# cg-tuwien/ppsurf

Measured on AMD Instinct MI355X. Metric: occupancy query-points/sec @ res=257, 50NN, higher is better.
Workload: dtype f16x3

## Files before the change

### include/ppsurf_amd_ext.h

```cpp
#ifndef PPSURF_AMD_EXT_H
#define PPSURF_AMD_EXT_H
#include <stddef.h>
#include <stdint.h>

#ifdef __cplusplus
extern "C" {
#endif

int ppsx_blend_rgba_u8(const int64_t* idx, const float* d2, int64_t m, int k, const uint8_t* rgba, int64_t n, double eps, uint8_t* out,
                       void* stream);

int ppsx_trim_cell_slots(const float* pts, int64_t n, const float* lo, const float* hi, float h, float inv_h, uint64_t* table, int64_t capacity,
                         int64_t* slot, void* stream);
int ppsx_trim_face_support(const float* verts, int64_t nv, const int64_t* faces, int64_t nf, const float* pts, int64_t n, const float* lo,
                           const float* hi, float h, float inv_h, const uint64_t* table, int64_t capacity, const int64_t* order,
                           const int64_t* offsets, double r, uint8_t* support, void* stream);

int ppsx_smooth_half_edges(const int64_t* faces, int64_t nf, int64_t nv, int64_t* keys, void* stream);
int ppsx_smooth_pass(const double* x, int64_t nv, const int64_t* offsets, const int32_t* nbr, const int32_t* mult, int64_t ne, double s,
                     double* out, void* stream);

int ppsx_normals_corner_keys(const int64_t* faces, int64_t nf, int64_t nv, int64_t* keys, void* stream);
int ppsx_normals_vertex(const float* verts, int64_t nv, const int64_t* faces, int64_t nf, const int64_t* offsets, const int32_t* inc, int64_t ni,
                        int weight, float* out, void* stream);
// ... 4 lines not shown
                       int64_t* keys, void* stream);
int ppsx_fill_loops(const int64_t* cand, int64_t nc, const int32_t* succ, int64_t nv, int max_edges, int32_t* len, void* stream);
int ppsx_fill_emit(const float* verts, int64_t nv, const int32_t* succ, const int64_t* leader, const int32_t* len, const int64_t* vslot,
                   const int64_t* foff, int64_t nl, float* new_verts, int64_t nnew, int64_t* new_faces, int64_t nfnew, void* stream);

int ppsx_denoise_face_normals(const float* verts, int64_t nv, const int64_t* faces, int64_t nf, double* normals, void* stream);
int ppsx_denoise_filter_pass(const int64_t* faces, int64_t nf, int64_t nv, const int64_t* offsets, const int32_t* inc, int64_t ni,
                             const double* normals, double threshold, double* out, void* stream);
int ppsx_denoise_vertex_pass(const double* x, int64_t nv, const int64_t* faces, int64_t nf, const double* normals, const int64_t* offsets,
                             const int32_t* inc, int64_t ni, double* out, void* stream);

int ppsx_pieces_edge_keys(const int64_t* faces, int64_t nf, int64_t nv, int64_t* keys, void* stream);
int ppsx_pieces_hook(const int32_t* fa, const int32_t* fb, int64_t np, int32_t* label, int64_t nf, int32_t* changed, void* stream);
int ppsx_pieces_compress(int32_t* label, int64_t nf, void* stream);
int ppsx_pieces_stats(const float* verts, int64_t nv, const int64_t* faces, int64_t nf, const int32_t* label, const int32_t* cid, int64_t nc,
                      int64_t* count, float* lo, float* hi, void* stream);
int ppsx_pieces_select(const int64_t* count, const float* lo, const float* hi, const int64_t* rank, int64_t nc, int has_min_faces,
                       int64_t min_faces, int has_min_diag_frac, double min_diag_frac, int has_keep_largest, int64_t keep_largest,
                       double box_diag2, uint8_t* keep, void* stream);

int ppsx_decimate_regular(const int64_t* offsets, const int32_t* mult, int64_t ne, const int64_t* inc_offsets, int64_t ni, int64_t nv,
                          uint8_t* regular, void* stream);
int ppsx_decimate_edges(const double* pos, int64_t nv, const int64_t* faces, int64_t nf, const int64_t* offsets, const int32_t* nbr,
                        const int32_t* src, int64_t ne, const int64_t* inc_offsets, const int32_t* inc, int64_t ni, const uint8_t* regular,
                        uint64_t* prio, double* x, uint8_t* fell, void* stream);
int ppsx_decimate_vertex_min(const int64_t* offsets, const int32_t* nbr, int64_t ne, int64_t nv, const uint64_t* prio, uint64_t* m1, void* stream);
int ppsx_decimate_ring_min(const int64_t* offsets, const int32_t* nbr, int64_t ne, int64_t nv, const uint64_t* m1, uint64_t* best, void* stream);
int ppsx_decimate_winners(const int32_t* src, const int32_t* nbr, int64_t ne, int64_t nv, const uint64_t* prio, const uint64_t* best, uint8_t* flag,
                          void* stream);
int ppsx_decimate_move(const int64_t* win, int64_t nw, const int32_t* src, const int32_t* nbr, int64_t ne, const double* x, double* pos, int64_t nv,
                       int32_t* rename, void* stream);
int ppsx_decimate_rename(const int64_t* faces, int64_t nf, int64_t nv, const int32_t* rename, int64_t* out, uint8_t* keep, void* stream);

#ifdef __cplusplus
}
#endif
#endif
```

### ppsurf_amd/csrc/pps_decode.hip

```cpp
#include <cstdlib>
#include "pps_common.h"
#include "../../include/ppsurf_amd.h"

using namespace pps;

#define NT 256
#define NW (NT / 64)
#define WG_PER_CU (512 / NT)
#ifndef PPS_PRIO
#define PPS_PRIO 1
#endif
#ifndef PPS_PRIO_PN
#define PPS_PRIO_PN 1
#endif
#define CH4 2048

template <int CHUNK_F4_NEXT, int NTH = NT, class F>
__device__ __forceinline__ void stream_step(const f32x4* __restrict__ gnext, f32x4*& cur, f32x4*& nxt, F&& compute) {
    chunk_copy_async<CHUNK_F4_NEXT / NTH, NTH>(gnext, nxt);
    compute((const f32x4*)cur);
    stream_wait();
    __syncthreads();
    f32x4* t = cur; cur = nxt; nxt = t;
}
// ... 1133 lines not shown
    f32x4 *cur, *nxt;
    stream_begin<CH4>(wg, cur, nxt);

    const int ntiles = (int)((Q + NW * 16 - 1) / (NW * 16));
    int first, count, stride;
    xcd_tile_range(ntiles, first, count, stride);
    for (int it = 0; it < count; ++it) {
        const TileRow q = tile_row(first + it * stride, wave, n, Q);
        f32x4 p[16], x[8], h[16];
        {
            const f32x4* sp = (const f32x4*)(pooled + q.c * 256) + g;
            const f32x4* sx = (const f32x4*)(xbar + q.c * 128) + g;
#pragma unroll
            for (int bb = 0; bb < 16; ++bb) p[bb] = sp[4 * bb];
#pragma unroll
            for (int bb = 0; bb < 8; ++bb) x[bb] = sx[4 * bb];
        }
#pragma unroll
        for (int c = 0; c < 8; ++c)
            stream_step<CH4>(wg + (c + 1) * CH4, cur, nxt,
                           [&](const f32x4* w) { dense_blocks<16, 2, 0>(p, &h[2 * c], w, bias4 + 8 * c, lane); });
#pragma unroll
        for (int c = 0; c < 4; ++c)
            stream_step<CH4>(wg + (c + 9) * CH4, cur, nxt,
                           [&](const f32x4* w) { dense_blocks<8, 4, 1, 1>(x, &h[4 * c], w, bias4, lane); });
#pragma unroll
        for (int c = 0; c < 8; ++c)
            stream_step<CH4>(wg + (c + 13) * CH4, cur, nxt,
                           [&](const f32x4* w) { dense_blocks<16, 2, 1>(h, &p[2 * c], w, bias4 + 64 + 8 * c, lane); });
        f32x4 o[2];
        stream_step<CH4>(wg, cur, nxt, [&](const f32x4* w) { dense_blocks<16, 2, 0>(p, o, w, bias4 + 128, lane); });
        store_logits(o[0], q, g, logits, occ);
    }
}

__global__ __launch_bounds__(NT, 2) void decode_tail_h_kernel(const float* __restrict__ pooled, const float* __restrict__ xbar, int64_t Q,
                                                              const f32x4* __restrict__ w16, const float* __restrict__ bias,
                                                              float* __restrict__ logits, float* __restrict__ occ, int* __restrict__ range) {
    float amax = 0.f;
    float* bias_l = (float*)((f32x4*)pps_smem + 2 * CH4);
    const f32x4* bias4 = (const f32x4*)bias_l;
    const f32x4* wg = w16;
    const int lane = lane_id(), wave = threadIdx.x >> 6, n = lane & 15, g = lane >> 4;

    lds_fill(bias_l, bias, TL_NBIAS);
    f32x4 *cur, *nxt;
    stream_begin<CH4>(wg, cur, nxt);

    const int ntiles = (int)((Q + NW * 16 - 1) / (NW * 16));
    int first, count, stride;
    xcd_tile_range(ntiles, first, count, stride);
    for (int it = 0; it < count; ++it) {
        const TileRow q = tile_row(first + it * stride, wave, n, Q);
        HiLo p[8], x[4];
        {
            const f32x4* sp = (const f32x4*)(pooled + q.c * 256) + g;
            const f32x4* sx = (const f32x4*)(xbar + q.c * 128) + g;
#pragma unroll
            for (int kb = 0; kb < 8; ++kb) p[kb] = split_f16_r(amax, sp[4 * (2 * kb)], sp[4 * (2 * kb + 1)]);
#pragma unroll
            for (int kb = 0; kb < 4; ++kb) x[kb] = split_f16_r(amax, sx[4 * (2 * kb)], sx[4 * (2 * kb + 1)]);
        }
        HiLo y[8];
#pragma unroll
        for (int c = 0; c < 8; ++c) {
            f32x4 h[2];
// ... 212 lines not shown
                        float* logits, float* occ, void* stream) {
    return decode_tail_f32_impl(pooled, xbar, q, wpack, bias, logits, occ, nullptr, stream);
}

int pps_decode_tail_f16x3(const float* pooled, const float* xbar, int64_t q, const void* w16, const float* bias, float* logits, float* occ,
                          int32_t* range_flag, void* stream) {
    if (q < 0) return PPS_ERR_ARG;
    if (q == 0) return PPS_OK;
    if (!pooled || !xbar || !w16 || !bias || !logits) return PPS_ERR_ARG;
    return launch<decode_tail_h_kernel>(grid_for((q + NW * 16 - 1) / (NW * 16)), NT, TL_LDS_BYTES, stream, pooled, xbar, q, (const f32x4*)w16, bias,
                                        logits, occ, (int*)range_flag);
}

#define PPS_DECODE_WS_HEAD 64
size_t pps_decode_ws_bytes(int64_t q) { return q < 0 ? 0 : (size_t)q * (256 + 256 + 4096 + 256) * sizeof(float) + PPS_DECODE_WS_HEAD; }

static int decode_fwd(const float* table, const float* pts, const float* query, const int64_t* idx, int64_t q, int k,
                      const float* patches, int p, const float* const* weights, float* logits, float* occ, void* ws, void* const* events,
                      void* stream, const void* const* w16 = nullptr) {
    const void* interp_w16 = w16 ? w16[0] : nullptr;
    const bool pn16 = w16 && w16[1] && w16[2] && w16[3];
    if (q < 0) return PPS_ERR_ARG;
    if (q == 0) return PPS_OK;
    if (!weights || !ws || !logits) return PPS_ERR_ARG;
    for (int i = 0; i < 10; ++i)
        if (!weights[i]) return PPS_ERR_ARG;
    int* guard = (int*)ws;
    float* pooled = (float*)ws + PPS_DECODE_WS_HEAD / sizeof(float);
    float* g = pooled + q * 256;
    float* trans2 = g + q * 256;
    float* xbar = trans2 + q * 4096;
    hipStream_t st = (hipStream_t)stream;
    const bool split = interp_w16 || pn16 || (w16 && w16[4]);
    if (split && hipMemsetAsync(guard, 0, sizeof(int), st) != hipSuccess) return PPS_ERR_LAUNCH;
#define PPS_MARK(i) do { if (events && events[i] && hipEventRecord((hipEvent_t)events[i], st) != hipSuccess) return PPS_ERR_LAUNCH; } while (0)
    PPS_MARK(0);
    int rc = interp_w16 ? pps_interp_pool_f16x3(table, pts, query, idx, q, k, weights[0], interp_w16, weights[1], pooled, guard, stream)
                        : pps_interp_pool_f32(table, pts, query, idx, q, k, weights[0], weights[1], pooled, stream);
    PPS_MARK(1);
    if (pn16) {
        if (rc == PPS_OK) rc = pps_pointnet_f16x3(patches, q, p, weights + 2, w16 + 1, g, trans2, xbar, guard, events ? events + 2 : nullptr, stream);
    } else {
        if (rc == PPS_OK) rc = pps_pointnet_stn_rows_f32(patches, q, p, weights[2], weights[3], g, stream);
        PPS_MARK(2);
        if (rc == PPS_OK) rc = pps_pointnet_stn_fc_f32(g, q, weights[4], weights[5], trans2, stream);
        PPS_MARK(3);
        if (rc == PPS_OK) rc = pps_pointnet_feat_rows_f32(patches, trans2, q, p, weights[6], weights[7], xbar, stream);
        PPS_MARK(4);
    }
    if (rc == PPS_OK)
        rc = (w16 && w16[4]) ? pps_decode_tail_f16x3(pooled, xbar, q, w16[4], weights[9], logits, occ, guard, stream)
                             : pps_decode_tail_f32(pooled, xbar, q, weights[8], weights[9], logits, occ, stream);
    PPS_MARK(5);
#undef PPS_MARK
    if (split && rc == PPS_OK) {
        rc = interp_pool_f32_impl(table, pts, query, idx, q, k, weights[0], weights[1], pooled, guard, stream);
        if (rc == PPS_OK) rc = launch_stn_rows<false>(patches, q, p, weights[2], weights[2] + PA_W_XYZ, weights[3], g, guard, stream);
        if (rc == PPS_OK) rc = stn_fc_f32_impl(g, q, weights[4], weights[5], trans2, guard, stream);
        if (rc == PPS_OK) rc = launch_feat_rows<false>(patches, trans2, q, p, weights[6], weights[6] + PC_W_XYZ, weights[7], xbar, guard, stream);
        if (rc == PPS_OK) rc = decode_tail_f32_impl(pooled, xbar, q, weights[8], weights[9], logits, occ, guard, stream);
    }
    return rc;
}

int pps_decode_fwd_f32(const float* table, const float* pts, const float* query, const int64_t* idx, int64_t q, int k,
                       const float* patches, int p, const float* const* weights, float* logits, float* occ, void* ws, void* stream) {
    return decode_fwd(table, pts, query, idx, q, k, patches, p, weights, logits, occ, ws, nullptr, stream);
// ... 17 lines not shown
```

### ppsurf_amd/csrc/pps_knn.hip

```cpp
#include "pps_common.h"
#include "../../include/ppsurf_amd.h"

#define KNN_QW 8
#define KNN_WAVES 4
#define KNN_CAP 128
#ifndef KNN_BISECT
#define KNN_BISECT 12
#endif
#ifndef KNN_SEED
#define KNN_SEED 4
#endif

typedef unsigned long long u64;

__device__ __forceinline__ u64 shfl_xor_u64(u64 v, int m) {
    const int lo = __shfl_xor((int)(unsigned)v, m), hi = __shfl_xor((int)(unsigned)(v >> 32), m);
    return ((u64)(unsigned)hi << 32) | (unsigned)lo;
}
__device__ __forceinline__ u64 shfl_u64(u64 v, int src) {
    const int lo = __shfl((int)(unsigned)v, src), hi = __shfl((int)(unsigned)(v >> 32), src);
    return ((u64)(unsigned)hi << 32) | (unsigned)lo;
}

__device__ __forceinline__ float wave_min_f32(float v, int lane) {
    v = fminf(v, pps::dpp_mov<0xB1>(v));
    v = fminf(v, pps::dpp_mov<0x4E>(v));
    v = fminf(v, pps::dpp_mov<0x141>(v));
    v = fminf(v, pps::dpp_mov<0x140>(v));
    v = fminf(v, __uint_as_float(pps::lane_xor_u32(__float_as_uint(v), 16, lane)));
    v = fminf(v, __uint_as_float(pps::lane_xor_u32(__float_as_uint(v), 32, lane)));
    return v;
}

__device__ __forceinline__ u64 wave_sort64(u64 key, int lane) {
#pragma unroll
    for (int size = 2; size <= 64; size <<= 1) {
#pragma unroll
        for (int st = size >> 1; st > 0; st >>= 1) {
            const u64 other = pps::lane_xor_u64(key, st, lane);
            const bool up = ((lane & size) == 0);
            const bool lower = ((lane & st) == 0);
            const bool take_min = (up == lower);
            const u64 mn = key < other ? key : other, mx = key < other ? other : key;
            key = take_min ? mn : mx;
        }
    }
    return key;
}
__device__ __forceinline__ u64 wave_bitonic_merge64(u64 key, int lane) {
#pragma unroll
    for (int st = 32; st > 0; st >>= 1) {
        const u64 other = pps::lane_xor_u64(key, st, lane);
        const bool lower = ((lane & st) == 0);
        const u64 mn = key < other ? key : other, mx = key < other ? other : key;
        key = lower ? mn : mx;
    }
    return key;
}

__device__ __forceinline__ u64 knn_flush(u64 list, const u64* cand, int cnt, int lane) {
    while (cnt > 0) {
        const int c = cnt < 64 ? cnt : 64;
        u64 ck = (lane < c) ? cand[cnt - c + lane] : ~0ull;
        ck = wave_sort64(ck, lane);
        const u64 rev = shfl_u64(ck, 63 - lane);
        list = wave_bitonic_merge64(list < rev ? list : rev, lane);
        cnt -= c;
    }
    return list;
}

__global__ __launch_bounds__(KNN_WAVES * 64) void knn_kernel(const float* __restrict__ pts, int n, const float* __restrict__ query,
                                                             int64_t m, int k, int64_t* __restrict__ out_idx,
                                                             float* __restrict__ out_d2) {
    __shared__ u64 cand_all[KNN_WAVES][KNN_QW][KNN_CAP];
    const int lane = threadIdx.x & 63, wave = threadIdx.x >> 6;
    const int64_t ntask = (m + KNN_QW - 1) / KNN_QW;
    for (int64_t task = (int64_t)blockIdx.x * KNN_WAVES + wave; task < ntask; task += (int64_t)gridDim.x * KNN_WAVES) {
        const int64_t q0 = task * KNN_QW;
        float qx[KNN_QW], qy[KNN_QW], qz[KNN_QW], tau[KNN_QW];
        u64 list[KNN_QW];
        int cnt[KNN_QW];
#pragma unroll
        for (int j = 0; j < KNN_QW; ++j) {
            const int64_t qq = (q0 + j < m) ? q0 + j : m - 1;
            qx[j] = __builtin_nontemporal_load(query + qq * 3);
            qy[j] = query[qq * 3 + 1];
            qz[j] = query[qq * 3 + 2];
// ... 26 lines not shown
                }
            }
        }
#pragma unroll
        for (int j = 0; j < KNN_QW; ++j) {
            list[j] = knn_flush(list[j], cand_all[wave][j], cnt[j], lane);
            if (q0 + j < m && lane < k) {
                out_idx[(q0 + j) * k + lane] = (int64_t)(unsigned)(list[j] & 0xffffffffull);
                if (out_d2) out_d2[(q0 + j) * k + lane] = __uint_as_float((unsigned)(list[j] >> 32));
            }
        }
    }
}

__device__ __forceinline__ void wave_merge2(u64& a, u64& b, int lane) {
    const u64 rev = shfl_u64(b, 63 - lane);
    const u64 lo = a < rev ? a : rev, hi = a < rev ? rev : a;
    a = wave_bitonic_merge64(lo, lane);
    b = wave_bitonic_merge64(hi, lane);
}

template <int R>
__device__ __forceinline__ void knn_flush_r(u64 (&list)[R], const u64* cand, int cnt, int lane) {
    while (cnt > 0) {
        const int c = cnt < 64 ? cnt : 64;
        u64 carry = (lane < c) ? cand[cnt - c + lane] : ~0ull;
        carry = wave_sort64(carry, lane);
#pragma unroll
        for (int r = 0; r < R; ++r) wave_merge2(list[r], carry, lane);
        cnt -= c;
    }
}

template <int R>
__global__ __launch_bounds__(KNN_WAVES * 64) void knn_blocked_kernel(const float* __restrict__ pts, const int* __restrict__ orig,
                                                                     const float* __restrict__ bbox, int nb,
                                                                     const float* __restrict__ win_bbox, int n_win,
                                                                     const float* __restrict__ sbox ,
                                                                     const float* __restrict__ query, int64_t m, int k,
                                                                     int64_t* __restrict__ out_idx, float* __restrict__ out_d2) {
    __shared__ u64 cand_all[KNN_WAVES][KNN_QW][KNN_CAP];
    const int ngrp = (nb + 63) >> 6;
    const int lane = threadIdx.x & 63, wave = threadIdx.x >> 6;
    const int kr = (k - 1) >> 6, kl = (k - 1) & 63;
    const int64_t ntask = (m + KNN_QW - 1) / KNN_QW;
    for (int64_t task = (int64_t)blockIdx.x * KNN_WAVES + wave; task < ntask; task += (int64_t)gridDim.x * KNN_WAVES) {
        const int64_t q0 = task * KNN_QW;
        float qx[KNN_QW], qy[KNN_QW], qz[KNN_QW], tau[KNN_QW];
        u64 list[KNN_QW][R];
        int cnt[KNN_QW], wbest[KNN_QW];
#pragma unroll
        for (int j = 0; j < KNN_QW; ++j) {
            const int64_t qq = (q0 + j < m) ? q0 + j : m - 1;
            qx[j] = __shfl(query[qq * 3], 0); qy[j] = __shfl(query[qq * 3 + 1], 0); qz[j] = __shfl(query[qq * 3 + 2], 0);
            tau[j] = INFINITY;
            wbest[j] = 0;
#pragma unroll
            for (int r = 0; r < R; ++r) list[j][r] = ~0ull;
            cnt[j] = 0;
        }
        if (sbox != nullptr && n_win > 0) {
#pragma unroll
            for (int j = 0; j < KNN_QW; ++j) {
                float best = INFINITY;
                int bw = 0;
                for (int g0 = 0; g0 * 64 < n_win; g0 += 64) {
                    const int g = g0 + lane;
                    const bool gv = g * 64 < n_win;
                    const float* gb = sbox + (int64_t)(gv ? g : 0) * 6;
                    const float gx = fmaxf(fmaxf(__fsub_rn(gb[0], qx[j]), __fsub_rn(qx[j], gb[3])), 0.f);
                    const float gy = fmaxf(fmaxf(__fsub_rn(gb[1], qy[j]), __fsub_rn(qy[j], gb[4])), 0.f);
                    const float gz = fmaxf(fmaxf(__fsub_rn(gb[2], qz[j]), __fsub_rn(qz[j], gb[5])), 0.f);
                    const float gnear = gv ? __fadd_rn(__fadd_rn(__fmul_rn(gx, gx), __fmul_rn(gy, gy)), __fmul_rn(gz, gz)) : INFINITY;
// ... 12 lines not shown
                        const float tf = wave_min_f32(far2, lane);
                        if (tf < best) {
                            best = tf;
                            bw = (g0 + src) * 64 + __builtin_ctzll(__ballot(far2 == tf));
                        }
                        pend &= ~(1ull << src);
                        pend &= __ballot(gnear < best);
                    }
                }
                tau[j] = best;
                wbest[j] = bw;
            }
        } else {
            for (int b0 = 0; b0 < n_win; b0 += 64) {
                const int b = b0 + lane;
                const bool bv = b < n_win;
                const float* bb = win_bbox + (int64_t)(bv ? b : 0) * 6;
                const float lx = bb[0], ly = bb[1], lz = bb[2], hx = bb[3], hy = bb[4], hz = bb[5];
#pragma unroll
                for (int j = 0; j < KNN_QW; ++j) {
                    const float fx = fmaxf(fabsf(__fsub_rn(qx[j], lx)), fabsf(__fsub_rn(qx[j], hx)));
                    const float fy = fmaxf(fabsf(__fsub_rn(qy[j], ly)), fabsf(__fsub_rn(qy[j], hy)));
                    const float fz = fmaxf(fabsf(__fsub_rn(qz[j], lz)), fabsf(__fsub_rn(qz[j], hz)));
                    const float far2 = bv ? __fadd_rn(__fadd_rn(__fmul_rn(fx, fx), __fmul_rn(fy, fy)), __fmul_rn(fz, fz)) : INFINITY;
                    if (far2 < tau[j]) { tau[j] = far2; wbest[j] = b; }
                }
            }
        }
        const int nfull = n_win > 0 ? n_win + R - 1 : 0;
        constexpr int SEEDS = KNN_SEED > R ? KNN_SEED : R;
        const int nseed = nfull < SEEDS ? nfull : SEEDS;
#pragma unroll
        for (int j = 0; j < KNN_QW; ++j) {
            const float t = wave_min_f32(tau[j], lane);
            const u64 who = __ballot(tau[j] == t);
            tau[j] = t;
            if (nseed > 0) {
                const int w = __shfl(wbest[j], who != 0ull ? __builtin_ctzll(who) : 0);
                int s0 = w - (nseed - R) / 2;
                s0 = s0 < 0 ? 0 : s0;
                s0 = s0 + nseed > nfull ? nfull - nseed : s0;
                unsigned u[SEEDS];
#pragma unroll
                for (int rr = 0; rr < SEEDS; ++rr) {
                    const int p = (s0 + (rr < nseed ? rr : 0)) * 64 + lane;
                    const float dx = __fsub_rn(qx[j], pts[3 * p]), dy = __fsub_rn(qy[j], pts[3 * p + 1]), dz = __fsub_rn(qz[j], pts[3 * p + 2]);
                    const float d2 = __fadd_rn(__fadd_rn(__fmul_rn(dx, dx), __fmul_rn(dy, dy)), __fmul_rn(dz, dz));
                    u[rr] = rr < nseed ? __float_as_uint(d2) : 0xffffffffu;
                }
                unsigned lo = 0u, hi = __float_as_uint(tau[j]);
                {
                    int c = 0;
#pragma unroll
                    for (int rr = 0; rr < SEEDS; ++rr) c += __popcll(__ballot(u[rr] <= hi));
                    if (c < k) lo = hi;
                }
#pragma unroll
                for (int it = 0; it < KNN_BISECT; ++it) {
                    const unsigned mid = lo + ((hi - lo) >> 1);
                    int c = 0;
#pragma unroll
                    for (int rr = 0; rr < SEEDS; ++rr) c += __popcll(__ballot(u[rr] <= mid));
                    if (c >= k) hi = mid; else lo = mid + (lo < hi ? 1u : 0u);
                }
                tau[j] = __uint_as_float(hi);
            }
        }
// ... 56 lines not shown
                    const float d2 = __fadd_rn(__fadd_rn(__fmul_rn(dx, dx), __fmul_rn(dy, dy)), __fmul_rn(dz, dz));
                    const bool pass = pv && (d2 <= tau[j]);
                    const u64 mask = __ballot(pass);
                    if (mask != 0ull) {
                        u64* cand = cand_all[wave][j];
                        const int pos = cnt[j] + (int)__builtin_amdgcn_mbcnt_hi((unsigned)(mask >> 32), __builtin_amdgcn_mbcnt_lo((unsigned)mask, 0));
                        if (pass) cand[pos] = ((u64)__float_as_uint(d2) << 32) | (unsigned)oi;
                        cnt[j] += __popcll(mask);
                        if (cnt[j] > KNN_CAP - 64) {
                            knn_flush_r<R>(list[j], cand + (cnt[j] - 64), 64, lane);
                            cnt[j] -= 64;
                            u64 kth = list[j][R - 1];
#pragma unroll
                            for (int r = 0; r + 1 < R; ++r) kth = (r == kr) ? list[j][r] : kth;
                            tau[j] = fminf(tau[j], __uint_as_float((unsigned)(shfl_u64(kth, kl) >> 32)));
                        }
                    }
                }
            }
          }
        }
#pragma unroll
        for (int j = 0; j < KNN_QW; ++j) {
            knn_flush_r<R>(list[j], cand_all[wave][j], cnt[j], lane);
            if (q0 + j < m) {
#pragma unroll
                for (int r = 0; r < R; ++r) {
                    const int e = r * 64 + lane;
                    if (e < k) {
                        out_idx[(q0 + j) * k + e] = (int64_t)(unsigned)(list[j][r] & 0xffffffffull);
                        if (out_d2) out_d2[(q0 + j) * k + e] = __uint_as_float((unsigned)(list[j][r] >> 32));
                    }
                }
            }
        }
    }
}

#define KBB_MAX 8
struct KbbKind {
    const float* pts; const int* orig; const float* bbox; const float* win; const float* query; const int* q_orig; int64_t* out;
    int64_t pts_stride, orig_stride, bbox_stride, win_stride, query_stride, qorig_stride, out_stride;
    int nb, n_win, m, k, groups, group_end;
};
struct KbbArgs { KbbKind kind[KBB_MAX]; int nkinds, nclouds; };

__global__ __launch_bounds__(KNN_WAVES * 64) void knn_blocked_batch_kernel(const KbbArgs a) {
    __shared__ u64 cand_all[KNN_WAVES][KNN_QW][KNN_CAP];
    const int lane = threadIdx.x & 63, wave = threadIdx.x >> 6;
    const int total = a.kind[a.nkinds - 1].group_end;
    for (int grp = blockIdx.x * KNN_WAVES + wave; grp < total; grp += gridDim.x * KNN_WAVES) {
        int t = 0;
        while (grp >= a.kind[t].group_end) ++t;
        const KbbKind& kd = a.kind[t];
        const int local = grp - (t == 0 ? 0 : a.kind[t - 1].group_end);
        const int cloud = local / kd.groups, q0 = (local % kd.groups) * KNN_QW;
        const float* __restrict__ pts = kd.pts + cloud * kd.pts_stride;
        const int* __restrict__ orig = kd.orig + cloud * kd.orig_stride;
        const float* __restrict__ bbox = kd.bbox + cloud * kd.bbox_stride;
        const float* __restrict__ win_bbox = kd.win + cloud * kd.win_stride;
        const float* __restrict__ query = kd.query + cloud * kd.query_stride;
        const int nb = kd.nb, n_win = kd.n_win, m = kd.m, k = kd.k;
        float qx[KNN_QW], qy[KNN_QW], qz[KNN_QW], tau[KNN_QW];
        u64 list[KNN_QW];
        int cnt[KNN_QW];
#pragma unroll
        for (int j = 0; j < KNN_QW; ++j) {
            const int qq = (q0 + j < m) ? q0 + j : m - 1;
            qx[j] = __shfl(query[qq * 3], 0); qy[j] = __shfl(query[qq * 3 + 1], 0); qz[j] = __shfl(query[qq * 3 + 2], 0);
// ... 117 lines not shown
}

int pps_knn_blocked_f32(const float* pts_blocked, const int32_t* orig_idx, const float* bbox, int64_t nb, int64_t n,
                        const float* win_bbox, int64_t n_win, const float* query, int64_t m, int k, int64_t* out_idx, float* out_d2,
                        void* stream) {
    return pps_knn_blocked_groups_f32(pts_blocked, orig_idx, bbox, nb, n, win_bbox, n_win, nullptr, query, m, k, out_idx, out_d2, stream);
}

int pps_knn_blocked_groups_f32(const float* pts_blocked, const int32_t* orig_idx, const float* bbox, int64_t nb, int64_t n,
                               const float* win_bbox, int64_t n_win, const float* group_bbox, const float* query, int64_t m, int k,
                               int64_t* out_idx, float* out_d2, void* stream) {
    if (n < 1 || nb < 1 || nb * 64 < n || (nb - 1) * 64 >= n || m < 0 || k < 1 || k > 256 || k > n || nb > 0x1ffffff || n_win < 0)
        return PPS_ERR_ARG;
    if (m == 0) return PPS_OK;
    if (!pts_blocked || !orig_idx || !bbox || !query || !out_idx || (n_win > 0 && !win_bbox)) return PPS_ERR_ARG;
    const int64_t ntask = (m + KNN_QW - 1) / KNN_QW;
    int64_t blocks = (ntask + KNN_WAVES - 1) / KNN_WAVES;
    int cus = pps_device_cu_count();
    if (cus <= 0) cus = 256;
    if (blocks > (int64_t)cus * 8) blocks = (int64_t)cus * 8;
    const dim3 grid((unsigned)blocks), block(KNN_WAVES * 64);
    hipStream_t st = (hipStream_t)stream;
    const int r = (k + 63) / 64;
#define PPS_KNN_LAUNCH(R) hipLaunchKernelGGL(knn_blocked_kernel<R>, grid, block, 0, st, pts_blocked, orig_idx, bbox, (int)nb, win_bbox, \
                                             (int)n_win, group_bbox, query, m, k, out_idx, out_d2)
    if (r == 1) PPS_KNN_LAUNCH(1);
    else if (r == 2) PPS_KNN_LAUNCH(2);
    else if (r == 3) PPS_KNN_LAUNCH(3);
    else PPS_KNN_LAUNCH(4);
#undef PPS_KNN_LAUNCH
    return hipGetLastError() == hipSuccess ? PPS_OK : PPS_ERR_LAUNCH;
}

int pps_knn_blocked_batch_f32(int nkinds, int64_t nclouds, const float* const* pts_blocked, const int32_t* const* orig_idx,
                              const float* const* bbox, const int64_t* nb, const float* const* win_bbox, const int64_t* n_win,
                              const float* const* query, const int32_t* const* q_orig, const int64_t* query_stride, const int64_t* m,
                              const int* k, int64_t* const* out_idx, void* stream) {
    if (nkinds < 1 || nkinds > KBB_MAX || nclouds < 1 || !pts_blocked || !orig_idx || !bbox || !nb || !win_bbox || !n_win || !query || !q_orig ||
        !query_stride || !m || !k || !out_idx)
        return PPS_ERR_ARG;
    KbbArgs a;
    int64_t total = 0;
    for (int t = 0; t < nkinds; ++t) {
        if (!pts_blocked[t] || !orig_idx[t] || !bbox[t] || !query[t] || !out_idx[t] || nb[t] < 1 || nb[t] > 0x1ffffff || m[t] < 1 || k[t] < 1 ||
            k[t] > 64 || n_win[t] < 0 || (n_win[t] > 0 && !win_bbox[t]) || query_stride[t] < m[t] * 3)
            return PPS_ERR_ARG;
        KbbKind& kd = a.kind[t];
        kd.pts = pts_blocked[t]; kd.orig = orig_idx[t]; kd.bbox = bbox[t]; kd.win = win_bbox[t] ? win_bbox[t] : bbox[t];
        kd.query = query[t]; kd.q_orig = q_orig[t]; kd.out = out_idx[t];
        kd.pts_stride = nb[t] * 64 * 3; kd.orig_stride = nb[t] * 64; kd.bbox_stride = nb[t] * 6; kd.win_stride = n_win[t] * 6;
        kd.query_stride = query_stride[t]; kd.qorig_stride = query_stride[t] / 3; kd.out_stride = m[t] * k[t];
        kd.nb = (int)nb[t]; kd.n_win = (int)n_win[t]; kd.m = (int)m[t]; kd.k = k[t];
        kd.groups = (int)((m[t] + KNN_QW - 1) / KNN_QW);
        total += nclouds * kd.groups;
        if (total > 0x7fffffff) return PPS_ERR_ARG;
        kd.group_end = (int)total;
    }
    for (int t = nkinds; t < KBB_MAX; ++t) { a.kind[t] = a.kind[nkinds - 1]; a.kind[t].group_end = (int)total; }
    a.nkinds = nkinds;
    a.nclouds = (int)nclouds;
    int64_t blocks = (total + KNN_WAVES - 1) / KNN_WAVES;
    int cus = pps_device_cu_count();
    if (cus <= 0) cus = 256;
    if (blocks > (int64_t)cus * 8) blocks = (int64_t)cus * 8;
    hipLaunchKernelGGL(knn_blocked_batch_kernel, dim3((unsigned)blocks), dim3(KNN_WAVES * 64), 0, (hipStream_t)stream, a);
    return hipGetLastError() == hipSuccess ? PPS_OK : PPS_ERR_LAUNCH;
// ... 14 lines not shown
```

### ppsurf_amd/decoder.py

```python
import ctypes

import numpy as np
import torch

from . import _lib

BN_EPS = 1e-5
C = 256
HEADS = 64


def _np64(t):
    if isinstance(t, torch.Tensor):
        t = t.detach().cpu().numpy()
    return np.asarray(t, dtype=np.float64)


def _fold_bn(w, b, sd, bn):
    scale = _np64(sd[bn + '.weight']) / np.sqrt(_np64(sd[bn + '.running_var']) + BN_EPS)
    return w * scale[:, None], (b - _np64(sd[bn + '.running_mean'])) * scale + _np64(sd[bn + '.bias'])


def _wb(sd, name):
    w = _np64(sd[name + '.weight'])
    return w.reshape(w.shape[0], -1), _np64(sd[name + '.bias'])


def pack_dense(w):
    w = np.ascontiguousarray(w, dtype=np.float32)
    out = np.empty(_lib.lib().pps_packed_dense_floats(w.shape[0], w.shape[1]), dtype=np.float32)
    _lib.call('pps_pack_dense_f32', w.ctypes.data, w.shape[0], w.shape[1], out.ctypes.data)
    return out

# ... 170 lines not shown
    LANE_MIN_CHUNKS = 4

    def __init__(self, plan: DecoderPlan, table, pts, raw, k: int, p: int, same_cloud: bool, max_chunk: int, overlap: bool = False, lanes=None):
        from . import ops
        import os
        self.ops, self.plan, self.table, self.pts, self.raw = ops, plan, table, pts, raw
        self.k, self.p, self.same_cloud, self.overlap = int(k), int(p), bool(same_cloud), bool(overlap)
        env = os.environ.get('PPS_CHUNK_LANES')
        self.lanes = int(env) if env else lanes
        self.max_chunk = int(max_chunk)
        self.idx, self.patches = [], []
        self.pidx = None if (same_cloud and self.p <= self.k) else []
        self._grow_buffers(2)
        self.blocks = self.ops.KnnBlocks(pts)
        self.raw_blocks = None if self.pidx is None else self.ops.KnnBlocks(raw)
        dev = plan.device
        self.side = torch.cuda.Stream(device=dev) if overlap else None
        self.lane_streams = []
        self.ready = [torch.cuda.Event() for _ in range(2)]
        self.free = [torch.cuda.Event() for _ in range(2)]
        self.n = 0

    def _grow_buffers(self, count):
        dev = self.plan.device
        while len(self.idx) < count:
            self.idx.append(torch.empty((self.max_chunk, self.k), dtype=torch.int64, device=dev))
            self.patches.append(torch.empty((self.max_chunk, self.p, 3), dtype=torch.float32, device=dev))
            if self.pidx is not None:
                self.pidx.append(torch.empty((self.max_chunk, self.p), dtype=torch.int64, device=dev))

    def _spatial(self, q, b):
        m = q.shape[0]
        idx = self.idx[b][:m]
        if self.pidx is not None and self.same_cloud and self.p > self.k:
            src = self.pidx[b][:m]
            self.raw_blocks.query(q, self.p, out=src)
            idx.copy_(src[:, :self.k])
        else:
            self.blocks.query(q, self.k, out=idx)
            src = idx
            if self.pidx is not None:
                src = self.pidx[b][:m]
                self.raw_blocks.query(q, self.p, out=src)
        self.ops.patch_normalize(self.raw, q, src, self.p, out=self.patches[b][:m])

    def _run_lanes(self, chunks, want_occ, lanes):
        dev = self.plan.device
        main = torch.cuda.current_stream(dev)
        while len(self.lane_streams) < lanes:
            self.lane_streams.append(torch.cuda.Stream(device=dev))
        self._grow_buffers(max(lanes, 2))
        out = [None] * len(chunks)
        for ln in range(lanes):
            st = self.lane_streams[ln]
            st.wait_stream(main)
            with torch.cuda.stream(st):
                for i in range(ln, len(chunks), lanes):
                    q = chunks[i]
                    m = q.shape[0]
                    self._spatial(q, ln)
                    out[i] = self.plan.decode(self.table, self.pts, q, self.idx[ln][:m], self.patches[ln][:m], want_occ=want_occ, lane=ln)
        for ln in range(lanes):
            main.wait_stream(self.lane_streams[ln])
        for lg, oc in out:
            lg.record_stream(main)
            if oc is not None:
# ... 88 lines not shown
```

### ppsurf_amd/ops.py

```python
import torch

from . import _lib


def knn_point_major(pts: torch.Tensor, query: torch.Tensor, k: int, return_d2: bool = False, out: torch.Tensor = None):
    _lib.need_device('knn_point_major', pts, query)
    pts = pts.contiguous().float()
    query = query.contiguous().float()
    m = query.shape[0]
    idx = out if out is not None else torch.empty((m, k), dtype=torch.int64, device=pts.device)
    assert idx.dtype == torch.int64 and idx.is_contiguous() and tuple(idx.shape) == (m, k)
    d2 = torch.empty((m, k), dtype=torch.float32, device=pts.device) if return_d2 else None
    _lib.call('pps_knn_f32', pts, pts.shape[0], query, m, int(k), idx, d2)
    return (idx, d2) if return_d2 else idx


def knn_batch_point_major(pts_list, query_list, k_list):
    import ctypes
    outs = []
    for s in range(0, len(pts_list), 64):
        ps, qs, ks = pts_list[s:s + 64], query_list[s:s + 64], k_list[s:s + 64]
        nt = len(ps)
        P, I64, I = ctypes.c_void_p * nt, ctypes.c_int64 * nt, ctypes.c_int * nt
        pts, qry, out, ns, ms, kk = P(), P(), P(), I64(), I64(), I()
# ... 90 lines not shown
        self.pts = torch.cat([sorted_pts, sorted_pts[-1:].expand(pad, 3)], dim=0).contiguous()
        self.orig = torch.cat([order.to(torch.int32), torch.full((pad,), -1, dtype=torch.int32, device=pts.device)]).contiguous()
        blk = self.pts.view(nb, 64, 3)
        self.bbox = torch.cat([blk.min(dim=1)[0], blk.max(dim=1)[0]], dim=1).contiguous()
        ng = (nb + 63) // 64
        bb = torch.cat([self.bbox, self.bbox[-1:].expand(ng * 64 - nb, 6)], dim=0).view(ng, 64, 6)
        self.gbox = torch.cat([bb[:, :, :3].min(dim=1)[0], bb[:, :, 3:].max(dim=1)[0]], dim=1).contiguous()
        self._win = {}
        self.groups = True

    def _windows(self, r: int):
        if r not in self._win:
            nfull = self.n // 64
            if nfull < r:
                self._win[r] = None
            else:
                lo, hi = self.bbox[:nfull, :3], self.bbox[:nfull, 3:]
                wl = lo.unfold(0, r, 1).min(dim=2)[0]
                wh = hi.unfold(0, r, 1).max(dim=2)[0]
                self._win[r] = torch.cat([wl, wh], dim=1).contiguous()
        return self._win[r]

    def query(self, query: torch.Tensor, k: int, return_d2: bool = False, out: torch.Tensor = None):
        query = query.contiguous().float()
        m = query.shape[0]
        idx = out if out is not None else torch.empty((m, k), dtype=torch.int64, device=query.device)
        assert idx.dtype == torch.int64 and idx.is_contiguous() and tuple(idx.shape) == (m, k)
        d2 = torch.empty((m, k), dtype=torch.float32, device=query.device) if return_d2 else None
        win = self._windows((int(k) + 63) // 64) if 1 <= int(k) <= 256 else None
        _lib.call('pps_knn_blocked_groups_f32', self.pts, self.orig, self.bbox, self.nb, self.n, win, win.shape[0] if win is not None else 0,
                  self.gbox if self.groups else None, query, m, int(k), idx, d2)
        return (idx, d2) if return_d2 else idx


def dilate_box(mask: torch.Tensor, r: int) -> torch.Tensor:
    assert mask.dtype == torch.bool and mask.dim() == 3 and mask.is_cuda
    src = mask.contiguous()
    dst, tmp = torch.empty_like(src), torch.empty_like(src)
    _lib.call('pps_dilate_box_u8', src, dst, tmp, src.shape[0], src.shape[1], src.shape[2], int(r))
    return dst


def grow_frontier(volume: torch.Tensor, neg: torch.Tensor, pos: torch.Tensor, to_see: torch.Tensor) -> torch.Tensor:
    assert volume.dtype == torch.float64 and volume.is_cuda and volume.is_contiguous()
    for m in (neg, pos, to_see):
        assert m.dtype == torch.bool and m.shape == volume.shape and m.is_contiguous()
    out = torch.empty_like(to_see)
    _lib.call('pps_grow_frontier_f64', volume, neg, pos, to_see, out, volume.numel())
    return out


def grow_band_todo(volume: torch.Tensor, band: torch.Tensor) -> torch.Tensor:
    assert volume.dtype == torch.float64 and volume.is_cuda and volume.is_contiguous() and band.dtype == torch.bool and band.is_contiguous()
    out = torch.empty_like(band)
    _lib.call('pps_grow_band_todo_f64', volume, band, out, volume.numel())
    return out


def marching_cubes(volume: torch.Tensor, level: float):
    import ctypes
    from . import mcubes
    assert volume.dtype == torch.float64 and volume.dim() == 3 and volume.is_cuda and volume.is_contiguous()
    L = _lib.lib()
    nx, ny, nz = volume.shape
    dev = volume.device
    tri, ntri, amb, tun_index, tun_cand = mcubes.device_tables(dev)
# ... 91 lines not shown
```

Measured before the change: 12.64 million.

## Fuse kNN query with patch normalization and self-reset decode guard

Adds a fused kNN kernel that, after finding the k nearest neighbours, directly writes normalized patch coordinates (offset from query, divided by the p-th neighbour radius). This replaces a separate patch_normalize launch and its re-read of the indices. It also makes the decode guard reset itself through a last-block atomic instead of a per-call memset, and tweaks wave min and bitonic sort to use 32-bit lane exchanges. These add complexity, and the guard reset changes cross-kernel synchronisation semantics.

Result: no change. 12.75 million, median of 6 (+0.9%).

```diff
diff --git a/include/ppsurf_amd_ext.h b/include/ppsurf_amd_ext.h
--- a/include/ppsurf_amd_ext.h
+++ b/include/ppsurf_amd_ext.h
@@ -60,6 +60,10 @@
                        int32_t* rename, void* stream);
 int ppsx_decimate_rename(const int64_t* faces, int64_t nf, int64_t nv, const int32_t* rename, int64_t* out, uint8_t* keep, void* stream);
 
+int ppsx_knn_blocked_patches_f32(const float* pts_blocked, const int32_t* orig_idx, const float* bbox, int64_t nb, int64_t n,
+                                 const float* win_bbox, int64_t n_win, const float* group_bbox, const float* query, int64_t m, int k,
+                                 int64_t* out_idx, float* out_d2, const float* raw, int p, float* out_patches, void* stream);
+
 #ifdef __cplusplus
 }
 #endif
diff --git a/ppsurf_amd/csrc/pps_decode.hip b/ppsurf_amd/csrc/pps_decode.hip
--- a/ppsurf_amd/csrc/pps_decode.hip
+++ b/ppsurf_amd/csrc/pps_decode.hip
@@ -1189,6 +1189,16 @@
         stream_step<CH4>(wg, cur, nxt, [&](const f32x4* w) { dense_blocks<16, 2, 0>(p, o, w, bias4 + 128, lane); });
         store_logits(o[0], q, g, logits, occ);
     }
+    if (gate != nullptr) {
+        __syncthreads();
+        if (threadIdx.x == 0) {
+            __threadfence();
+            if (atomicAdd(gate + 2, 1) == (int)gridDim.x - 1) {
+                atomicExch(gate + 2, 0);
+                atomicExch(gate, 0);
+            }
+        }
+    }
 }
 
 __global__ __launch_bounds__(NT, 2) void decode_tail_h_kernel(const float* __restrict__ pooled, const float* __restrict__ xbar, int64_t Q,
@@ -1467,7 +1477,6 @@
     float* xbar = trans2 + q * 4096;
     hipStream_t st = (hipStream_t)stream;
     const bool split = interp_w16 || pn16 || (w16 && w16[4]);
-    if (split && hipMemsetAsync(guard, 0, sizeof(int), st) != hipSuccess) return PPS_ERR_LAUNCH;
 #define PPS_MARK(i) do { if (events && events[i] && hipEventRecord((hipEvent_t)events[i], st) != hipSuccess) return PPS_ERR_LAUNCH; } while (0)
     PPS_MARK(0);
     int rc = interp_w16 ? pps_interp_pool_f16x3(table, pts, query, idx, q, k, weights[0], interp_w16, weights[1], pooled, guard, stream)
diff --git a/ppsurf_amd/csrc/pps_knn.hip b/ppsurf_amd/csrc/pps_knn.hip
--- a/ppsurf_amd/csrc/pps_knn.hip
+++ b/ppsurf_amd/csrc/pps_knn.hip
@@ -1,5 +1,6 @@
 #include "pps_common.h"
 #include "../../include/ppsurf_amd.h"
+#include "../../include/ppsurf_amd_ext.h"
 
 #define KNN_QW 8
 #define KNN_WAVES 4
@@ -22,14 +23,25 @@
     return ((u64)(unsigned)hi << 32) | (unsigned)lo;
 }
 
-__device__ __forceinline__ float wave_min_f32(float v, int lane) {
-    v = fminf(v, pps::dpp_mov<0xB1>(v));
-    v = fminf(v, pps::dpp_mov<0x4E>(v));
-    v = fminf(v, pps::dpp_mov<0x141>(v));
-    v = fminf(v, pps::dpp_mov<0x140>(v));
-    v = fminf(v, __uint_as_float(pps::lane_xor_u32(__float_as_uint(v), 16, lane)));
-    v = fminf(v, __uint_as_float(pps::lane_xor_u32(__float_as_uint(v), 32, lane)));
-    return v;
+__device__ __forceinline__ float pps_uniform_f32(float v) {
+    return __uint_as_float((unsigned)__builtin_amdgcn_readfirstlane((int)__float_as_uint(v)));
+}
+
+__device__ __forceinline__ float wave_min_f32(float vf, int lane) {
+    unsigned v = __float_as_uint(vf);
+    v = min(v, pps::dpp_mov_u32<0xB1>(v));
+    v = min(v, pps::dpp_mov_u32<0x4E>(v));
+    v = min(v, pps::dpp_mov_u32<0x141>(v));
+    v = min(v, pps::dpp_mov_u32<0x140>(v));
+    v = min(v, pps::lane_xor_u32(v, 16, lane));
+    v = min(v, pps::lane_xor_u32(v, 32, lane));
+    return __uint_as_float(v);
+}
+
+__device__ __forceinline__ u64 key_lane_xor(u64 v, int st, int lane) {
+    typedef unsigned u32x2 __attribute__((ext_vector_type(2)));
+    const u32x2 w = __builtin_bit_cast(u32x2, v);
+    return __builtin_bit_cast(u64, u32x2{pps::lane_xor_u32(w.x, st, lane), pps::lane_xor_u32(w.y, st, lane)});
 }
 
 __device__ __forceinline__ u64 wave_sort64(u64 key, int lane) {
@@ -37,12 +49,11 @@
     for (int size = 2; size <= 64; size <<= 1) {
 #pragma unroll
         for (int st = size >> 1; st > 0; st >>= 1) {
-            const u64 other = pps::lane_xor_u64(key, st, lane);
+            const u64 other = key_lane_xor(key, st, lane);
             const bool up = ((lane & size) == 0);
             const bool lower = ((lane & st) == 0);
             const bool take_min = (up == lower);
-            const u64 mn = key < other ? key : other, mx = key < other ? other : key;
-            key = take_min ? mn : mx;
+            key = ((key < other) == take_min) ? key : other;
         }
     }
     return key;
@@ -50,10 +61,9 @@
 __device__ __forceinline__ u64 wave_bitonic_merge64(u64 key, int lane) {
 #pragma unroll
     for (int st = 32; st > 0; st >>= 1) {
-        const u64 other = pps::lane_xor_u64(key, st, lane);
+        const u64 other = key_lane_xor(key, st, lane);
         const bool lower = ((lane & st) == 0);
-        const u64 mn = key < other ? key : other, mx = key < other ? other : key;
-        key = lower ? mn : mx;
+        key = ((key < other) == lower) ? key : other;
     }
     return key;
 }
@@ -146,13 +156,14 @@
     }
 }
 
-template <int R>
-__global__ __launch_bounds__(KNN_WAVES * 64) void knn_blocked_kernel(const float* __restrict__ pts, const int* __restrict__ orig,
-                                                                     const float* __restrict__ bbox, int nb,
-                                                                     const float* __restrict__ win_bbox, int n_win,
-                                                                     const float* __restrict__ sbox ,
-                                                                     const float* __restrict__ query, int64_t m, int k,
-                                                                     int64_t* __restrict__ out_idx, float* __restrict__ out_d2) {
+template <int R, bool PATCH>
+__device__ __forceinline__ void knn_blocked_body(const float* __restrict__ pts, const int* __restrict__ orig, const float* __restrict__ bbox, int nb,
+                                                 const float* __restrict__ win_bbox, int n_win,
+                                                 const float* __restrict__ sbox ,
+                                                 const float* __restrict__ query, int64_t m, int k, int64_t* __restrict__ out_idx,
+                                                 float* __restrict__ out_d2, const float* __restrict__ raw ,
+                                                 int n_raw, int p_patch, float* __restrict__ patches) {
+    static_assert(!PATCH || R == 1, "the patch epilogue reads the whole list from one register");
     __shared__ u64 cand_all[KNN_WAVES][KNN_QW][KNN_CAP];
     const int ngrp = (nb + 63) >> 6;
     const int lane = threadIdx.x & 63, wave = threadIdx.x >> 6;
@@ -231,7 +242,7 @@
         const int nseed = nfull < SEEDS ? nfull : SEEDS;
 #pragma unroll
         for (int j = 0; j < KNN_QW; ++j) {
-            const float t = wave_min_f32(tau[j], lane);
+            const float t = pps_uniform_f32(wave_min_f32(tau[j], lane));
             const u64 who = __ballot(tau[j] == t);
             tau[j] = t;
             if (nseed > 0) {
@@ -354,9 +365,40 @@
                         if (out_d2) out_d2[(q0 + j) * k + e] = __uint_as_float((unsigned)(list[j][r] >> 32));
                     }
                 }
-            }
-        }
-    }
+                if constexpr (PATCH) {
+                    const u64 key = list[j][0];
+                    const float radius = __fsqrt_rn(__uint_as_float((unsigned)__builtin_amdgcn_readlane((int)(unsigned)(key >> 32), p_patch - 1)));
+                    const unsigned oi = (unsigned)key;
+                    if (lane < p_patch && oi < (unsigned)n_raw) {
+                        const float* rp = raw + (size_t)oi * 3;
+                        float* o = patches + ((q0 + j) * p_patch + lane) * 3;
+                        o[0] = __fdiv_rn(__fsub_rn(rp[0], qx[j]), radius);
+                        o[1] = __fdiv_rn(__fsub_rn(rp[1], qy[j]), radius);
+                        o[2] = __fdiv_rn(__fsub_rn(rp[2], qz[j]), radius);
+                    }
+                }
+            }
+        }
+    }
+}
+
+template <int R>
+__global__ __launch_bounds__(KNN_WAVES * 64) void knn_blocked_kernel(const float* __restrict__ pts, const int* __restrict__ orig,
+                                                                     const float* __restrict__ bbox, int nb,
+                                                                     const float* __restrict__ win_bbox, int n_win,
+                                                                     const float* __restrict__ sbox ,
+                                                                     const float* __restrict__ query, int64_t m, int k,
+                                                                     int64_t* __restrict__ out_idx, float* __restrict__ out_d2) {
+    knn_blocked_body<R, false>(pts, orig, bbox, nb, win_bbox, n_win, sbox, query, m, k, out_idx, out_d2, nullptr, 0, 0, nullptr);
+}
+
+__global__ __launch_bounds__(KNN_WAVES * 64) __attribute__((amdgpu_waves_per_eu(4, 4)))
+void knn_blocked_patches_kernel(const float* __restrict__ pts, const int* __restrict__ orig, const float* __restrict__ bbox, int nb,
+                                const float* __restrict__ win_bbox, int n_win, const float* __restrict__ sbox,
+                                const float* __restrict__ query, int64_t m, int k, int64_t* __restrict__ out_idx,
+                                float* __restrict__ out_d2, const float* __restrict__ raw, int n_raw, int p_patch,
+                                float* __restrict__ patches) {
+    knn_blocked_body<1, true>(pts, orig, bbox, nb, win_bbox, n_win, sbox, query, m, k, out_idx, out_d2, raw, n_raw, p_patch, patches);
 }
 
 #define KBB_MAX 8
@@ -540,6 +582,23 @@
     return hipGetLastError() == hipSuccess ? PPS_OK : PPS_ERR_LAUNCH;
 }
 
+int ppsx_knn_blocked_patches_f32(const float* pts_blocked, const int32_t* orig_idx, const float* bbox, int64_t nb, int64_t n,
+                                 const float* win_bbox, int64_t n_win, const float* group_bbox, const float* query, int64_t m, int k,
+                                 int64_t* out_idx, float* out_d2, const float* raw, int p, float* out_patches, void* stream) {
+    if (n < 1 || nb < 1 || nb * 64 < n || (nb - 1) * 64 >= n || m < 0 || k < 1 || k > 64 || k > n || p < 1 || p > k || nb > 0x1ffffff || n_win < 0)
+        return PPS_ERR_ARG;
+    if (m == 0) return PPS_OK;
+    if (!pts_blocked || !orig_idx || !bbox || !query || !out_idx || !raw || !out_patches || (n_win > 0 && !win_bbox)) return PPS_ERR_ARG;
+    const int64_t ntask = (m + KNN_QW - 1) / KNN_QW;
+    int64_t blocks = (ntask + KNN_WAVES - 1) / KNN_WAVES;
+    int cus = pps_device_cu_count();
+    if (cus <= 0) cus = 256;
+    if (blocks > (int64_t)cus * 8) blocks = (int64_t)cus * 8;
+    hipLaunchKernelGGL(knn_blocked_patches_kernel, dim3((unsigned)blocks), dim3(KNN_WAVES * 64), 0, (hipStream_t)stream, pts_blocked, orig_idx,
+                       bbox, (int)nb, win_bbox, (int)n_win, group_bbox, query, m, k, out_idx, out_d2, raw, (int)n, p, out_patches);
+    return hipGetLastError() == hipSuccess ? PPS_OK : PPS_ERR_LAUNCH;
+}
+
 int pps_knn_blocked_batch_f32(int nkinds, int64_t nclouds, const float* const* pts_blocked, const int32_t* const* orig_idx,
                               const float* const* bbox, const int64_t* nb, const float* const* win_bbox, const int64_t* n_win,
                               const float* const* query, const int32_t* const* q_orig, const int64_t* query_stride, const int64_t* m,
diff --git a/ppsurf_amd/decoder.py b/ppsurf_amd/decoder.py
--- a/ppsurf_amd/decoder.py
+++ b/ppsurf_amd/decoder.py
@@ -1,4 +1,5 @@
 import ctypes
+import os
 
 import numpy as np
 import torch
@@ -235,6 +236,9 @@
     def _spatial(self, q, b):
         m = q.shape[0]
         idx = self.idx[b][:m]
+        if self.pidx is None and self.k <= 64 and os.environ.get('PPS_SPATIAL_FUSED') != '0':
+            self.blocks.query_patches(q, self.k, self.raw, self.p, out=idx, out_patches=self.patches[b][:m])
+            return
         if self.pidx is not None and self.same_cloud and self.p > self.k:
             src = self.pidx[b][:m]
             self.raw_blocks.query(q, self.p, out=src)
diff --git a/ppsurf_amd/ops.py b/ppsurf_amd/ops.py
--- a/ppsurf_amd/ops.py
+++ b/ppsurf_amd/ops.py
@@ -146,6 +146,19 @@
                   self.gbox if self.groups else None, query, m, int(k), idx, d2)
         return (idx, d2) if return_d2 else idx
 
+    def query_patches(self, query: torch.Tensor, k: int, raw: torch.Tensor, p: int, out: torch.Tensor = None, out_patches: torch.Tensor = None):
+        query = query.contiguous().float()
+        m = query.shape[0]
+        idx = out if out is not None else torch.empty((m, k), dtype=torch.int64, device=query.device)
+        patches = out_patches if out_patches is not None else torch.empty((m, p, 3), dtype=torch.float32, device=query.device)
+        assert idx.dtype == torch.int64 and idx.is_contiguous() and tuple(idx.shape) == (m, k)
+        assert patches.dtype == torch.float32 and patches.is_contiguous() and tuple(patches.shape) == (m, p, 3)
+        assert raw.dtype == torch.float32 and raw.is_contiguous() and tuple(raw.shape) == (self.n, 3)
+        win = self._windows(1) if 1 <= int(k) <= 64 else None
+        _lib.call('ppsx_knn_blocked_patches_f32', self.pts, self.orig, self.bbox, self.nb, self.n, win, win.shape[0] if win is not None else 0,
+                  self.gbox if self.groups else None, query, m, int(k), idx, None, raw, int(p), patches)
+        return idx, patches
+
 
 def dilate_box(mask: torch.Tensor, r: int) -> torch.Tensor:
     assert mask.dtype == torch.bool and mask.dim() == 3 and mask.is_cuda
```
